# peterhpark/neuroclear

Hardware: AMD Instinct MI355X
Metric: voxels/sec (higher is better)
Workload: dtype f32

## Files before the change

### neuroclear_amd/csrc/norm_act.hip

```cpp
#include <cstdlib>

#include "common.hpp"
#include "s3_common.hpp"

namespace nc {

static constexpr int kMaxSplits = 64;

static int pick_splits(int NC, long S) {
  long want = cdiv(2048, NC);
  long cap = cdiv(S, 8192);
  long s = want < cap ? want : cap;
  if (s < 1) s = 1;
  if (s > kMaxSplits) s = kMaxSplits;
  return (int)s;
}

__device__ __forceinline__ void block_reduce2(double& a, double& b, double* out2) {
  __shared__ double red[2][4];
  for (int o = 32; o > 0; o >>= 1) {
    a += __shfl_down(a, o);
    b += __shfl_down(b, o);
  }
  const int lane = threadIdx.x & 63, wv = threadIdx.x >> 6;
// ... 2 lines not shown
    red[1][wv] = b;
  }
  __syncthreads();
  if (threadIdx.x == 0) {
    out2[0] = (red[0][0] + red[0][1]) + (red[0][2] + red[0][3]);
    out2[1] = (red[1][0] + red[1][1]) + (red[1][2] + red[1][3]);
  }
}

__device__ __forceinline__ void chunk_range(long S, int splits, int sp, long& b, long& e) {
  long chunk = (S + splits - 1) / splits;
  chunk = (chunk + 3) & ~3L;
  b = (long)sp * chunk;
  e = b + chunk < S ? b + chunk : S;
  if (b > S) b = S;
}

__global__ __launch_bounds__(256) void k_in_stats(const float* __restrict__ x, long S, int splits,
                                                  double* __restrict__ part) {
  const int inst = blockIdx.y, sp = blockIdx.x;
  long b, e;
  chunk_range(S, splits, sp, b, e);
  const float* p = x + (long)inst * S;
  double s = 0.0, q = 0.0;
  if ((S & 3) == 0 && ((uintptr_t)x & 15) == 0) {
    const float4* p4 = reinterpret_cast<const float4*>(p);
    for (long i = b / 4 + threadIdx.x; i < e / 4; i += 256) {
      const float4 v = p4[i];
      const double a0 = v.x, a1 = v.y, a2 = v.z, a3 = v.w;
      s += (a0 + a1) + (a2 + a3);
      q = fma(a0, a0, q); q = fma(a1, a1, q); q = fma(a2, a2, q); q = fma(a3, a3, q);
    }
  } else {
    for (long i = b + threadIdx.x; i < e; i += 256) {
      const double a = p[i];
      s += a;
      q = fma(a, a, q);
    }
  }
  block_reduce2(s, q, part + ((long)inst * splits + sp) * 2);
}

__global__ void k_in_finalize(const double* __restrict__ part, int NC, int splits, long S, float eps,
                              float* __restrict__ mean, float* __restrict__ rstd) {
  const int i = blockIdx.x * blockDim.x + threadIdx.x;
  if (i >= NC) return;
  double s = 0.0, q = 0.0;
  for (int k = 0; k < splits; ++k) {
    s += part[((long)i * splits + k) * 2];
    q += part[((long)i * splits + k) * 2 + 1];
  }
  const double m = s / (double)S;
  double var = q / (double)S - m * m;
  if (var < 0.0) var = 0.0;
  mean[i] = (float)m;
  rstd[i] = (float)(1.0 / sqrt(var + (double)eps));
}

__global__ __launch_bounds__(256) void k_in_act_fwd(const float* __restrict__ x, const float* __restrict__ mean,
                                                    const float* __restrict__ rstd, float slope,
                                                    float* __restrict__ y, long S) {
  const int inst = blockIdx.y;
  const float m = mean[inst], r = rstd[inst];
  const float* p = x + (long)inst * S;
  float* o = y + (long)inst * S;
  if ((S & 3) == 0 && (((uintptr_t)x | (uintptr_t)y) & 15) == 0) {
    const float4* p4 = reinterpret_cast<const float4*>(p);
    float4* o4 = reinterpret_cast<float4*>(o);
    for (long i = (long)blockIdx.x * 256 + threadIdx.x; i < S / 4; i += (long)gridDim.x * 256) {
      float4 v = p4[i];
      v.x = (v.x - m) * r; v.y = (v.y - m) * r; v.z = (v.z - m) * r; v.w = (v.w - m) * r;
      v.x = v.x > 0.f ? v.x : v.x * slope; v.y = v.y > 0.f ? v.y : v.y * slope;
      v.z = v.z > 0.f ? v.z : v.z * slope; v.w = v.w > 0.f ? v.w : v.w * slope;
      o4[i] = v;
    }
  } else {
    for (long i = (long)blockIdx.x * 256 + threadIdx.x; i < S; i += (long)gridDim.x * 256) {
      const float v = (p[i] - m) * r;
      o[i] = v > 0.f ? v : v * slope;
    }
  }
}

__global__ __launch_bounds__(256) void k_in_bwd_sums(const float* __restrict__ dy, const float* __restrict__ x,
                                                     const float* __restrict__ mean, const float* __restrict__ rstd,
                                                     float slope, long S, int splits, double* __restrict__ part) {
  const int inst = blockIdx.y, sp = blockIdx.x;
  long b, e;
  chunk_range(S, splits, sp, b, e);
  const float m = mean[inst], r = rstd[inst];
  const float* px = x + (long)inst * S;
  const float* pg = dy + (long)inst * S;
  double s1 = 0.0, s2 = 0.0;
  for (long i = b + threadIdx.x; i < e; i += 256) {
    const float xh = (px[i] - m) * r;
    const float g = xh > 0.f ? pg[i] : pg[i] * slope;
    s1 += (double)g;
    s2 = fma((double)g, (double)xh, s2);
  }
  block_reduce2(s1, s2, part + ((long)inst * splits + sp) * 2);
}

__device__ __forceinline__ float in_bwd_value(float xv, float gy, float m, float r, float m1, float m2, float slope) {
  const float xh = (xv - m) * r;
  const float g = xh > 0.f ? gy : gy * slope;
  float p = xh * m2;
  asm("" : "+v"(p));
  return r * ((g - m1) - p);
}

__global__ __launch_bounds__(256) void k_in_bwd_apply(const float* __restrict__ dy, const float* __restrict__ x,
                                                      const float* __restrict__ mean, const float* __restrict__ rstd,
                                                      float slope, long S, int splits,
                                                      const double* __restrict__ part, float* __restrict__ dx,
                                                      double* __restrict__ rowpart) {
  const int inst = blockIdx.y;
  double s1 = 0.0, s2 = 0.0;
  for (int k = 0; k < splits; ++k) {
    s1 += part[((long)inst * splits + k) * 2];
    s2 += part[((long)inst * splits + k) * 2 + 1];
  }
  const float m1 = (float)(s1 / (double)S), m2 = (float)(s2 / (double)S);
  const float m = mean[inst], r = rstd[inst];
  const float* px = x + (long)inst * S;
  const float* pg = dy + (long)inst * S;
  float* o = dx + (long)inst * S;
  double rs = 0.0;
  for (long i = (long)blockIdx.x * 256 + threadIdx.x; i < S; i += (long)gridDim.x * 256) {
    const float v = in_bwd_value(px[i], pg[i], m, r, m1, m2, slope);
    o[i] = v;
    rs += (double)v;
  }
  if (rowpart) {
    double zero = 0.0, out2[2];
    block_reduce2(rs, zero, out2);
    if (threadIdx.x == 0) rowpart[(long)inst * gridDim.x + blockIdx.x] = out2[0];
  }
}

__global__ __launch_bounds__(256) void k_in_dbias_final(const double* __restrict__ rowpart, int N, int C, int nb,
                                                        float* __restrict__ dbias) {
  const int c = blockIdx.x;
  double s = 0.0, zero = 0.0;
  const int total = N * nb;
  for (int i = threadIdx.x; i < total; i += 256) {
    const int n = i / nb, b = i - n * nb;
    s += rowpart[((long)n * C + c) * nb + b];
  }
  __shared__ double out2[2];
  block_reduce2(s, zero, out2);
  if (threadIdx.x == 0) dbias[c] = (float)out2[0];
}

static constexpr long kRowsMaxS = 2048;

template <int G>
__device__ __forceinline__ double group_sum(double v) {
#pragma unroll
  for (int o = G / 2; o > 0; o >>= 1) v += __shfl_xor(v, o);
  return v;
}

template <int G, int MODE>
__global__ __launch_bounds__(256) void k_in_fwd_rows(const float* __restrict__ x, long NC, int S, float eps, float slope,
                                                     float* __restrict__ mean, float* __restrict__ rstd,
                                                     float* __restrict__ y) {
  const int sub = threadIdx.x % G;
  const long inst = (long)blockIdx.x * (256 / G) + threadIdx.x / G;
  if (inst >= NC) return;
  const float* p = x + inst * S;
  float m, r;
  if constexpr (MODE != 1) {
    double s = 0.0, q = 0.0;
#pragma unroll 4
    for (int i = sub; i < S; i += G) {
      const double a = p[i];
      s += a;
      q = fma(a, a, q);
    }
    s = group_sum<G>(s);
    q = group_sum<G>(q);
    const double mm = s / (double)S;
    double var = q / (double)S - mm * mm;
    if (var < 0.0) var = 0.0;
    m = (float)mm;
    r = (float)(1.0 / sqrt(var + (double)eps));
    if (sub == 0) {
      mean[inst] = m;
      rstd[inst] = r;
    }
  } else {
    m = mean[inst];
    r = rstd[inst];
  }
  if constexpr (MODE != 0) {
    float* o = y + inst * S;
#pragma unroll 4
    for (int i = sub; i < S; i += G) {
      const float v = (p[i] - m) * r;
      o[i] = v > 0.f ? v : v * slope;
    }
  }
}

template <int G>
__global__ __launch_bounds__(256) void k_in_bwd_rows(const float* __restrict__ dy, const float* __restrict__ x,
                                                     const float* __restrict__ mean, const float* __restrict__ rstd,
                                                     float slope, long NC, int S, float* __restrict__ dx,
                                                     double* __restrict__ rowsum) {
  const int sub = threadIdx.x % G;
  const long inst = (long)blockIdx.x * (256 / G) + threadIdx.x / G;
// ... 135 lines not shown
  if (rowpart) {
    const int lane = threadIdx.x & 63, wv = threadIdx.x >> 6;
#pragma unroll
    for (int j = 0; j < 8; ++j) {
      double a = rs[j];
      for (int of = 32; of > 0; of >>= 1) a += __shfl_down(a, of);
      if (lane == 0) red[j][wv] = a;
    }
    __syncthreads();
    if (threadIdx.x < 8)
      rowpart[(ncb * 8 + threadIdx.x) * gridDim.x + blockIdx.x] =
          (red[threadIdx.x][0] + red[threadIdx.x][1]) + (red[threadIdx.x][2] + red[threadIdx.x][3]);
  }
}

__device__ __forceinline__ float r1_product(float w, float s) {
  float g = __builtin_fmaf(w, s, 0.f);
  asm("" : "+v"(g));
  return g;
}

template <bool R1 = false>
__global__ __launch_bounds__(256) void k_in_bwd_apply_s3(const float* __restrict__ dy, const float* __restrict__ x,
                                                         const float* __restrict__ mean, const float* __restrict__ rstd,
                                                         float slope, long S, int splits, const double* __restrict__ part,
                                                         uint4* __restrict__ dxs, int cblocks, double* __restrict__ rowpart,
                                                         const unsigned* __restrict__ guard = nullptr, const float* __restrict__ w1 = nullptr) {
  __shared__ float sm[2][8];
  __shared__ double red[8][4];
  if (guard_skip(guard, 1)) return;
  const long ncb = blockIdx.y;
  if (threadIdx.x < 8) {
    const long inst = ncb * 8 + threadIdx.x;
    double s1 = 0.0, s2 = 0.0;
    for (int k = 0; k < splits; ++k) {
      s1 += part[(inst * splits + k) * 2];
      s2 += part[(inst * splits + k) * 2 + 1];
    }
    sm[0][threadIdx.x] = (float)(s1 / (double)S);
    sm[1][threadIdx.x] = (float)(s2 / (double)S);
  }
  __syncthreads();
  float m[8], r[8], m1[8], m2[8];
#pragma unroll
  for (int j = 0; j < 8; ++j) { m[j] = mean[ncb * 8 + j]; r[j] = rstd[ncb * 8 + j]; m1[j] = sm[0][j]; m2[j] = sm[1][j]; }
  const float* px = x + ncb * 8 * S;
  const float* pg = R1 ? dy : dy + ncb * 8 * S;
  float wj[8];
#pragma unroll
  for (int j = 0; j < 8; ++j) wj[j] = R1 ? w1[ncb * 8 + j] : 0.f;
  double rs[8];
#pragma unroll
  for (int j = 0; j < 8; ++j) rs[j] = 0.0;
  for (long v = (long)blockIdx.x * 256 + threadIdx.x; v < S; v += (long)gridDim.x * 256) {
    unsigned short e[8][3];
    const float sv = R1 ? pg[v] : 0.f;
#pragma unroll
    for (int j = 0; j < 8; ++j) {
      const float t = in_bwd_value(px[j * S + v], R1 ? r1_product(wj[j], sv) : pg[j * S + v], m[j], r[j], m1[j], m2[j], slope);
      rs[j] += (double)t;
      s3_split(t, e[j]);
    }
#pragma unroll
    for (int t = 0; t < 3; ++t) dxs[(ncb * 3 + t) * S + v] = s3_unit(e, t);
  }
  if (rowpart) {
    const int lane = threadIdx.x & 63, wv = threadIdx.x >> 6;
#pragma unroll
    for (int j = 0; j < 8; ++j) {
      double a = rs[j];
      for (int of = 32; of > 0; of >>= 1) a += __shfl_down(a, of);
      if (lane == 0) red[j][wv] = a;
    }
    __syncthreads();
    if (threadIdx.x < 8)
      rowpart[(ncb * 8 + threadIdx.x) * gridDim.x + blockIdx.x] =
          (red[threadIdx.x][0] + red[threadIdx.x][1]) + (red[threadIdx.x][2] + red[threadIdx.x][3]);
  }
}

template <bool R1 = false>
__global__ __launch_bounds__(256) void k_in_bwd_sums_h2(const float* __restrict__ dy, const float* __restrict__ x, const float* __restrict__ mean,
                                                        const float* __restrict__ rstd, float slope, long S, int splits,
                                                        double* __restrict__ part, unsigned* __restrict__ gmax, unsigned* __restrict__ xmax,
                                                        const float* __restrict__ w1 = nullptr) {
  const int inst = blockIdx.y, sp = blockIdx.x;
  long b, e;
  chunk_range(S, splits, sp, b, e);
  const float m = mean[inst], r = rstd[inst];
  const float* px = x + (long)inst * S;
  const float* pg = R1 ? dy : dy + (long)inst * S;
  const float w = R1 ? w1[inst] : 0.f;
  double s1 = 0.0, s2 = 0.0;
  unsigned gm = 0, xm = 0;
  for (long i = b + threadIdx.x; i < e; i += 256) {
    const float xh = (px[i] - m) * r;
    const float gy = R1 ? r1_product(w, pg[i]) : pg[i];
    const float g = xh > 0.f ? gy : gy * slope;
    s1 += (double)g;
    s2 = fma((double)g, (double)xh, s2);
    const unsigned gb = __float_as_uint(g) & 0x7fffffffu, xb = __float_as_uint(xh) & 0x7fffffffu;
    if (gb < 0x7f800000u && gb > gm) gm = gb;
    if (xb < 0x7f800000u && xb > xm) xm = xb;
  }
#pragma unroll
  for (int o = 32; o > 0; o >>= 1) {
    const unsigned q1 = (unsigned)__shfl_xor((int)gm, o), q2 = (unsigned)__shfl_xor((int)xm, o);
    gm = q1 > gm ? q1 : gm; xm = q2 > xm ? q2 : xm;
  }
  if ((threadIdx.x & 63) == 0) {
    if (gm) atomicMax(gmax + inst, gm);
    if (xm) atomicMax(xmax + inst, xm);
  }
  block_reduce2(s1, s2, part + ((long)inst * splits + sp) * 2);
}

__global__ __launch_bounds__(256) void k_in_bwd_bound(const float* __restrict__ rstd, const unsigned* __restrict__ gmax,
                                                      const unsigned* __restrict__ xmax, int NC, unsigned* __restrict__ cell,
                                                      unsigned* __restrict__ cell2, unsigned* __restrict__ guard) {
  if (guard && threadIdx.x < 8) guard[threadIdx.x] = 0u;
  unsigned m = 0;
  for (int i = threadIdx.x; i < NC; i += 256) {
    const float bnd = rstd[i] * __uint_as_float(gmax[i]) * (2.f + __uint_as_float(xmax[i]));
    const unsigned b = __float_as_uint(bnd) & 0x7fffffffu;
    if (b < 0x7f800000u && b > m) m = b;
  }
#pragma unroll
  for (int o = 32; o > 0; o >>= 1) {
    const unsigned q = (unsigned)__shfl_xor((int)m, o);
    m = q > m ? q : m;
  }
  if ((threadIdx.x & 63) == 0 && m) {
    atomicMax(cell, m);
    atomicMax(cell2, m);
  }
}

__global__ void k_zero_u32(unsigned* p, int n) {
  for (int i = blockIdx.x * blockDim.x + threadIdx.x; i < n; i += gridDim.x * blockDim.x) p[i] = 0u;
}

template <bool R1 = false>
__global__ __launch_bounds__(256) void k_in_bwd_apply_h2(const float* __restrict__ dy, const float* __restrict__ x,
                                                         const float* __restrict__ mean, const float* __restrict__ rstd,
                                                         float slope, long S, int splits, const double* __restrict__ part,
                                                         uint4* __restrict__ dxs, int cblocks, double* __restrict__ rowpart,
                                                         const unsigned* __restrict__ cell, unsigned* __restrict__ guard,
                                                         const float* __restrict__ w1 = nullptr) {
  __shared__ float sm[2][8];
  __shared__ double red[8][4];
  const long ncb = blockIdx.y;
  if (threadIdx.x < 8) {
    const long inst = ncb * 8 + threadIdx.x;
    double s1 = 0.0, s2 = 0.0;
    for (int k = 0; k < splits; ++k) {
      s1 += part[(inst * splits + k) * 2];
      s2 += part[(inst * splits + k) * 2 + 1];
    }
    sm[0][threadIdx.x] = (float)(s1 / (double)S);
    sm[1][threadIdx.x] = (float)(s2 / (double)S);
  }
  __syncthreads();
  const unsigned cbits = *cell;
  const float sc = h2_scale(cbits);
  unsigned n_zero = 0, n_low = 0;
  float m[8], r[8], m1[8], m2[8];
#pragma unroll
  for (int j = 0; j < 8; ++j) { m[j] = mean[ncb * 8 + j]; r[j] = rstd[ncb * 8 + j]; m1[j] = sm[0][j]; m2[j] = sm[1][j]; }
  const float* px = x + ncb * 8 * S;
  const float* pg = R1 ? dy : dy + ncb * 8 * S;
  float wj[8];
#pragma unroll
  for (int j = 0; j < 8; ++j) wj[j] = R1 ? w1[ncb * 8 + j] : 0.f;
  double rs[8];
#pragma unroll
  for (int j = 0; j < 8; ++j) rs[j] = 0.0;
  for (long v = (long)blockIdx.x * 256 + threadIdx.x; v < S; v += (long)gridDim.x * 256) {
    unsigned short e[8][3];
    unsigned mx = 0;
    const float sv = R1 ? pg[v] : 0.f;
#pragma unroll
    for (int j = 0; j < 8; ++j) {
      float t = in_bwd_value(px[j * S + v], R1 ? r1_product(wj[j], sv) : pg[j * S + v], m[j], r[j], m1[j], m2[j], slope);
      rs[j] += (double)t;
      asm("" : "+v"(t));
      const unsigned b = __float_as_uint(t) & 0x7fffffffu;
      if (b < 0x7f800000u && b > mx) mx = b;
      h2_split(t * sc, e[j]);
    }
#pragma unroll
    for (int t = 0; t < 2; ++t) dxs[(ncb * 2 + t) * S + v] = s3_unit(e, t);
    if (guard) {
      const unsigned thr = cbits > kGuardDrop ? cbits - kGuardDrop : 0u;
      const bool any_hi = __builtin_amdgcn_ballot_w64(mx >= thr && mx != 0) != 0;
      const bool any_nz = __builtin_amdgcn_ballot_w64(mx != 0) != 0;
      if (!any_nz) ++n_zero;
      else if (!any_hi) ++n_low;
    }
  }
  if (guard && (threadIdx.x & 63) == 0) {
    if (n_low) atomicAdd(guard + kGuardLow, n_low);
    if (n_zero) atomicAdd(guard + kGuardAll, n_zero);
  }
  if (rowpart) {
    const int lane = threadIdx.x & 63, wv = threadIdx.x >> 6;
#pragma unroll
    for (int j = 0; j < 8; ++j) {
      double a = rs[j];
      for (int of = 32; of > 0; of >>= 1) a += __shfl_down(a, of);
      if (lane == 0) red[j][wv] = a;
    }
    __syncthreads();
    if (threadIdx.x < 8)
      rowpart[(ncb * 8 + threadIdx.x) * gridDim.x + blockIdx.x] =
          (red[threadIdx.x][0] + red[threadIdx.x][1]) + (red[threadIdx.x][2] + red[threadIdx.x][3]);
  }
}


__global__ void k_lrelu_fwd(const float* __restrict__ x, float slope, float* __restrict__ y, long n) {
  for (long i = (long)blockIdx.x * blockDim.x + threadIdx.x; i < n; i += (long)gridDim.x * blockDim.x) {
    const float v = x[i];
    y[i] = v > 0.f ? v : v * slope;
  }
}
__global__ void k_lrelu_bwd(const float* __restrict__ dy, const float* __restrict__ x, float slope,
                            float* __restrict__ dx, long n) {
  for (long i = (long)blockIdx.x * blockDim.x + threadIdx.x; i < n; i += (long)gridDim.x * blockDim.x)
    dx[i] = x[i] > 0.f ? dy[i] : dy[i] * slope;
}
__global__ void __launch_bounds__(256) k_in_act_tail(const float* __restrict__ x, const float* __restrict__ mean, const float* __restrict__ rstd,
                                                     const float* __restrict__ w1, const float* __restrict__ b1, const float* __restrict__ w2,
                                                     const float* __restrict__ b2, float* __restrict__ y, long S, int C) {
  __shared__ float sm[3][256];
  for (int c = threadIdx.x; c < C; c += 256) { sm[0][c] = mean[c]; sm[1][c] = rstd[c]; sm[2][c] = w1[c]; }
  __syncthreads();
  const long v = (long)blockIdx.x * 256 + threadIdx.x;
  if (v >= S) return;
  float acc = 0.f;
  for (int c = 0; c < C; ++c) {
    float t = (x[(long)c * S + v] - sm[0][c]) * sm[1][c];
    t = t > 0.f ? t : 0.f;
    acc = fmaf(sm[2][c], t, acc);
  }
  const float t1 = acc + b1[0];
  const float t2 = fmaf(w2[0], t1, b2[0]);
// ... 186 lines not shown
                      void* stream) {
  if (!x || !mean || !rstd) { set_error("instnorm_stats: null pointer"); return NC_ERR_ARG; }
  if (NC >= 1 && S >= 1 && rows_path(S)) {
    launch_fwd_rows<0>(x, NC, S, eps, 0.f, mean, rstd, nullptr, (hipStream_t)stream);
    return check_launch("instnorm_stats");
  }
  if (NC > 65535) {
    for (int c0 = 0; c0 < NC; c0 += 65535) {
      const int n = NC - c0 < 65535 ? NC - c0 : 65535;
      if (int e = nc_instnorm_stats(x + (long)c0 * S, n, S, eps, mean + c0, rstd + c0, ws, ws_bytes, stream)) return e;
    }
    return NC_OK;
  }
  if (NC < 1 || S < 1) { set_error("instnorm_stats: bad shape NC=%d S=%ld", NC, S); return NC_ERR_SHAPE; }
  if (!ws || ws_bytes < nc_instnorm_ws_bytes(NC, S)) { set_error("instnorm_stats: workspace too small"); return NC_ERR_WS; }
  hipStream_t s = (hipStream_t)stream;
  const int splits = pick_splits(NC, S);
  hipLaunchKernelGGL(k_in_stats, dim3(splits, NC), dim3(256), 0, s, x, S, splits, (double*)ws);
  hipLaunchKernelGGL(k_in_finalize, dim3((unsigned)cdiv(NC, 128)), dim3(128), 0, s, (const double*)ws, NC, splits, S, eps,
                     mean, rstd);
  return check_launch("instnorm_stats");
}

int nc_instnorm_act_fwd(const float* x, const float* mean, const float* rstd, float slope, float* y, int NC, long S,
                        void* stream) {
  if (!x || !mean || !rstd || !y) { set_error("instnorm_act_fwd: null pointer"); return NC_ERR_ARG; }
  if (NC >= 1 && S >= 1 && rows_path(S)) {
    launch_fwd_rows<1>(x, NC, S, 0.f, slope, const_cast<float*>(mean), const_cast<float*>(rstd), y, (hipStream_t)stream);
    return check_launch("instnorm_act_fwd");
  }
  if (NC > 65535) {
    for (int c0 = 0; c0 < NC; c0 += 65535) {
      const int n = NC - c0 < 65535 ? NC - c0 : 65535;
      if (int e = nc_instnorm_act_fwd(x + (long)c0 * S, mean + c0, rstd + c0, slope, y + (long)c0 * S, n, S, stream)) return e;
    }
    return NC_OK;
  }
  if (NC < 1 || S < 1) { set_error("instnorm_act_fwd: bad shape"); return NC_ERR_SHAPE; }
  long bx = cdiv(S, 1024 * 4);
  if (bx > 1024) bx = 1024;
  hipLaunchKernelGGL(k_in_act_fwd, dim3((unsigned)bx, NC), dim3(256), 0, (hipStream_t)stream, x, mean, rstd, slope, y, S);
  return check_launch("instnorm_act_fwd");
}

int nc_instnorm_fwd(const float* x, float eps, float slope, float* mean, float* rstd, float* y, int NC, long S, void* ws,
                    size_t ws_bytes, void* stream) {
  if (!x || !mean || !rstd || !y) { set_error("instnorm_fwd: null pointer"); return NC_ERR_ARG; }
  if (NC < 1 || S < 1) { set_error("instnorm_fwd: bad shape NC=%d S=%ld", NC, S); return NC_ERR_SHAPE; }
  if (rows_path(S)) {
    launch_fwd_rows<2>(x, NC, S, eps, slope, mean, rstd, y, (hipStream_t)stream);
    return check_launch("instnorm_fwd");
  }
  if (int e = nc_instnorm_stats(x, NC, S, eps, mean, rstd, ws, ws_bytes, stream)) return e;
  return nc_instnorm_act_fwd(x, mean, rstd, slope, y, NC, S, stream);
}

int nc_instnorm_act_bwd(const float* dy, const float* x, const float* mean, const float* rstd, float slope, float* dx,
                        int NC, long S, void* ws, size_t ws_bytes, void* stream) {
  if (!dy || !x || !mean || !rstd || !dx) { set_error("instnorm_act_bwd: null pointer"); return NC_ERR_ARG; }
  if (NC >= 1 && S >= 1 && rows_path(S)) {
    launch_bwd_rows(dy, x, mean, rstd, slope, NC, S, dx, nullptr, (hipStream_t)stream);
    return check_launch("instnorm_act_bwd");
  }
  if (NC > 65535) {
    for (int c0 = 0; c0 < NC; c0 += 65535) {
      const int n = NC - c0 < 65535 ? NC - c0 : 65535;
      if (int e = nc_instnorm_act_bwd(dy + (long)c0 * S, x + (long)c0 * S, mean + c0, rstd + c0, slope, dx + (long)c0 * S, n, S, ws,
                                      ws_bytes, stream)) return e;
    }
    return NC_OK;
  }
  if (NC < 1 || S < 1) { set_error("instnorm_act_bwd: bad shape"); return NC_ERR_SHAPE; }
  if (!ws || ws_bytes < nc_instnorm_ws_bytes(NC, S)) { set_error("instnorm_act_bwd: workspace too small"); return NC_ERR_WS; }
  hipStream_t s = (hipStream_t)stream;
  const int splits = pick_splits(NC, S);
  hipLaunchKernelGGL(k_in_bwd_sums, dim3(splits, NC), dim3(256), 0, s, dy, x, mean, rstd, slope, S, splits, (double*)ws);
  long bx = cdiv(S, 1024);
  if (bx > 1024) bx = 1024;
  hipLaunchKernelGGL(k_in_bwd_apply, dim3((unsigned)bx, NC), dim3(256), 0, s, dy, x, mean, rstd, slope, S, splits,
                     (const double*)ws, dx, (double*)nullptr);
  return check_launch("instnorm_act_bwd");
}

size_t nc_instnorm_bwd_dbias_ws_bytes(int NC, long S) {
  long bx = cdiv(S, 1024);
  if (bx > 1024) bx = 1024;
  return nc_instnorm_ws_bytes(NC, S) + (size_t)NC * bx * sizeof(double);
}

int nc_instnorm_act_bwd_dbias(const float* dy, const float* x, const float* mean, const float* rstd, float slope, float* dx,
                              float* dbias, int N, int C, long S, void* ws, size_t ws_bytes, void* stream) {
  if (!dy || !x || !mean || !rstd || !dx || !dbias) { set_error("instnorm_act_bwd_dbias: null pointer"); return NC_ERR_ARG; }
  const long NCl = (long)N * C;
  if (N < 1 || C < 1 || S < 1 || NCl > 0x7fffffffL) { set_error("instnorm_act_bwd_dbias: bad shape"); return NC_ERR_SHAPE; }
  hipStream_t s = (hipStream_t)stream;
  if (rows_path(S)) {
    if (!ws || ws_bytes < (size_t)NCl * sizeof(double)) { set_error("instnorm_act_bwd_dbias: workspace too small"); return NC_ERR_WS; }
    launch_bwd_rows(dy, x, mean, rstd, slope, NCl, S, dx, (double*)ws, s);
    hipLaunchKernelGGL(k_in_dbias_final, dim3(C), dim3(256), 0, s, (const double*)ws, N, C, 1, dbias);
    return check_launch("instnorm_act_bwd_dbias");
  }
  if (NCl > 65535) { set_error("instnorm_act_bwd_dbias: more than 65535 long instances"); return NC_ERR_SHAPE; }
  const int NC = (int)NCl;
  if (!ws || ws_bytes < nc_instnorm_bwd_dbias_ws_bytes(NC, S)) { set_error("instnorm_act_bwd_dbias: workspace too small"); return NC_ERR_WS; }
  const int splits = pick_splits(NC, S);
  double* rowpart = (double*)((char*)ws + nc_instnorm_ws_bytes(NC, S));
  hipLaunchKernelGGL(k_in_bwd_sums, dim3(splits, NC), dim3(256), 0, s, dy, x, mean, rstd, slope, S, splits, (double*)ws);
  long bx = cdiv(S, 1024);
  if (bx > 1024) bx = 1024;
  hipLaunchKernelGGL(k_in_bwd_apply, dim3((unsigned)bx, NC), dim3(256), 0, s, dy, x, mean, rstd, slope, S, splits,
                     (const double*)ws, dx, rowpart);
  hipLaunchKernelGGL(k_in_dbias_final, dim3(C), dim3(256), 0, s, (const double*)rowpart, N, C, (int)bx, dbias);
  return check_launch("instnorm_act_bwd_dbias");
}

int nc_instnorm_act_fwd_c8(const float* x, const float* mean, const float* rstd, float slope, float* y, void* yh, int N, int C,
                           long S, int dtype, void* stream) {
  if (!x || !mean || !rstd || !yh) { set_error("instnorm_act_fwd_c8: null pointer"); return NC_ERR_ARG; }
  if (N < 1 || C < 8 || C % 8 || S < 1 || (long)N * C / 8 > 65535) { set_error("instnorm_act_fwd_c8: bad shape"); return NC_ERR_SHAPE; }
  if (dtype != NC_DT_F16 && dtype != NC_DT_BF16) { set_error("instnorm_act_fwd_c8: dtype must be NC_DT_F16 or NC_DT_BF16"); return NC_ERR_ARG; }
  long bx = cdiv(S, 256);
  if (bx > 2048) bx = 2048;
  dim3 grid((unsigned)bx, (unsigned)(N * C / 8));
  if (dtype == NC_DT_F16)
    hipLaunchKernelGGL(k_in_act_fwd_c8<NC_DT_F16>, grid, dim3(256), 0, (hipStream_t)stream, x, mean, rstd, slope, y, (uint4*)yh, S);
  else
    hipLaunchKernelGGL(k_in_act_fwd_c8<NC_DT_BF16>, grid, dim3(256), 0, (hipStream_t)stream, x, mean, rstd, slope, y, (uint4*)yh, S);
  return check_launch("instnorm_act_fwd_c8");
}

int nc_instnorm_act_bwd_c8(const float* dy, const float* x, const float* mean, const float* rstd, float slope, float* dx,
                           void* dxh, float* dbias, int N, int C, long S, int dtype, void* ws, size_t ws_bytes, void* stream) {
  if (!dy || !x || !mean || !rstd || !dx || !dxh) { set_error("instnorm_act_bwd_c8: null pointer"); return NC_ERR_ARG; }
  const long NCl = (long)N * C;
  if (N < 1 || C < 8 || C % 8 || S < 1 || NCl > 65535) { set_error("instnorm_act_bwd_c8: bad shape"); return NC_ERR_SHAPE; }
  if (dtype != NC_DT_F16 && dtype != NC_DT_BF16) { set_error("instnorm_act_bwd_c8: dtype must be NC_DT_F16 or NC_DT_BF16"); return NC_ERR_ARG; }
  const int NC = (int)NCl;
  if (!ws || ws_bytes < nc_instnorm_bwd_dbias_ws_bytes(NC, S)) { set_error("instnorm_act_bwd_c8: workspace too small"); return NC_ERR_WS; }
  hipStream_t s = (hipStream_t)stream;
  const int splits = pick_splits(NC, S);
  hipLaunchKernelGGL(k_in_bwd_sums, dim3(splits, NC), dim3(256), 0, s, dy, x, mean, rstd, slope, S, splits, (double*)ws);
  long bx = cdiv(S, 1024);
  if (bx > 1024) bx = 1024;
  double* rowpart = dbias ? (double*)((char*)ws + nc_instnorm_ws_bytes(NC, S)) : nullptr;
  dim3 grid((unsigned)bx, (unsigned)(NC / 8));
  if (dtype == NC_DT_F16)
    hipLaunchKernelGGL(k_in_bwd_apply_c8<NC_DT_F16>, grid, dim3(256), 0, s, dy, x, mean, rstd, slope, S, splits,
                       (const double*)ws, dx, (uint4*)dxh, rowpart);
  else
    hipLaunchKernelGGL(k_in_bwd_apply_c8<NC_DT_BF16>, grid, dim3(256), 0, s, dy, x, mean, rstd, slope, S, splits,
                       (const double*)ws, dx, (uint4*)dxh, rowpart);
  if (dbias) hipLaunchKernelGGL(k_in_dbias_final, dim3(C), dim3(256), 0, s, (const double*)rowpart, N, C, (int)bx, dbias);
  return check_launch("instnorm_act_bwd_c8");
}

}
namespace nc {
bool instnorm_bwd_s3_supported(int N, int C, long S) { return N >= 1 && C >= 8 && C % 8 == 0 && S >= 1 && !rows_path(S) && (long)N * C <= 65535; }
int instnorm_act_bwd_dbias_s3(const float* dy, const float* x, const float* mean, const float* rstd, float slope, void* dxs,
                              float* dbias, int N, int C, long S, void* ws, size_t ws_bytes, void* stream) {
  if (!dy || !x || !mean || !rstd || !dxs || !dbias) { set_error("instnorm_act_bwd_dbias_s3: null pointer"); return NC_ERR_ARG; }
  if (!instnorm_bwd_s3_supported(N, C, S)) { set_error("instnorm_act_bwd_dbias_s3: bad shape"); return NC_ERR_SHAPE; }
  const int NC = N * C;
  if (!ws || ws_bytes < nc_instnorm_bwd_dbias_ws_bytes(NC, S)) { set_error("instnorm_act_bwd_dbias_s3: workspace too small"); return NC_ERR_WS; }
  hipStream_t s = (hipStream_t)stream;
  const int splits = pick_splits(NC, S);
  hipLaunchKernelGGL(k_in_bwd_sums, dim3(splits, NC), dim3(256), 0, s, dy, x, mean, rstd, slope, S, splits, (double*)ws);
  long bx = cdiv(S, 1024);
  if (bx > 1024) bx = 1024;
  double* rowpart = (double*)((char*)ws + nc_instnorm_ws_bytes(NC, S));
  hipLaunchKernelGGL(k_in_bwd_apply_s3<false>, dim3((unsigned)bx, (unsigned)(NC / 8)), dim3(256), 0, s, dy, x, mean, rstd, slope, S, splits,
                     (const double*)ws, (uint4*)dxs, C / 8, rowpart, (const unsigned*)nullptr, (const float*)nullptr);
  hipLaunchKernelGGL(k_in_dbias_final, dim3(C), dim3(256), 0, s, (const double*)rowpart, N, C, (int)bx, dbias);
  return check_launch("instnorm_act_bwd_dbias_s3");
}
static int in_bwd_dbias_h2(const float* dy, const float* w1, const float* x, const float* mean, const float* rstd, float slope, void* dxs,
                           float* dbias, int N, int C, long S, void* ws, size_t ws_bytes, void* stream, unsigned* guard) {
  if (!dy || !x || !mean || !rstd || !dxs || !dbias) { set_error("instnorm_act_bwd_dbias_h2: null pointer"); return NC_ERR_ARG; }
  if (!instnorm_bwd_s3_supported(N, C, S)) { set_error("instnorm_act_bwd_dbias_h2: bad shape"); return NC_ERR_SHAPE; }
  const int NC = N * C;
  if (w1 && N != 1) { set_error("instnorm_act_bwd_dbias_h2: the rank-one form takes one sample"); return NC_ERR_ARG; }
  if (!ws || ws_bytes < nc_instnorm_bwd_dbias_ws_bytes(NC, S)) { set_error("instnorm_act_bwd_dbias_h2: workspace too small"); return NC_ERR_WS; }
  if ((size_t)NC * S * 2 < 512 + (size_t)NC * 8) { set_error("instnorm_act_bwd_dbias_h2: tensor too small"); return NC_ERR_SHAPE; }
  hipStream_t s = (hipStream_t)stream;
  unsigned* cells = (unsigned*)((char*)dxs + h2_cells_offset((size_t)NC * S));
  unsigned* gmax = cells + 64;
  unsigned* xmax = gmax + NC;
  hipLaunchKernelGGL(k_zero_u32, dim3((unsigned)cdiv(64 + 2 * NC, 256)), dim3(256), 0, s, cells, 64 + 2 * NC);
  const int splits = pick_splits(NC, S);
  if (w1)
    hipLaunchKernelGGL(k_in_bwd_sums_h2<true>, dim3(splits, NC), dim3(256), 0, s, dy, x, mean, rstd, slope, S, splits, (double*)ws, gmax, xmax, w1);
  else
    hipLaunchKernelGGL(k_in_bwd_sums_h2<false>, dim3(splits, NC), dim3(256), 0, s, dy, x, mean, rstd, slope, S, splits, (double*)ws, gmax, xmax,
                       (const float*)nullptr);
  hipLaunchKernelGGL(k_in_bwd_bound, dim3(1), dim3(256), 0, s, rstd, gmax, xmax, NC, cells, cells + 1, guard);
  long bx = cdiv(S, 1024);
  if (bx > 1024) bx = 1024;
  double* rowpart = (double*)((char*)ws + nc_instnorm_ws_bytes(NC, S));
  unsigned* g = guard && h2_guard_on() ? guard : nullptr;
  if (w1)
    hipLaunchKernelGGL(k_in_bwd_apply_h2<true>, dim3((unsigned)bx, (unsigned)(NC / 8)), dim3(256), 0, s, dy, x, mean, rstd, slope, S, splits,
                       (const double*)ws, (uint4*)dxs, C / 8, rowpart, (const unsigned*)cells, g, w1);
  else
    hipLaunchKernelGGL(k_in_bwd_apply_h2<false>, dim3((unsigned)bx, (unsigned)(NC / 8)), dim3(256), 0, s, dy, x, mean, rstd, slope, S, splits,
                       (const double*)ws, (uint4*)dxs, C / 8, rowpart, (const unsigned*)cells, g, (const float*)nullptr);
  hipLaunchKernelGGL(k_in_dbias_final, dim3(C), dim3(256), 0, s, (const double*)rowpart, N, C, (int)bx, dbias);
  if (g) {
    const unsigned long long total = (unsigned long long)(NC / 8) * (unsigned long long)cdiv(S, 64);
    const bool flip = h2_guard_can_flip();
    if (int e = h2_guard_decide(g, nullptr, nullptr, g + kGuardFlag, flip, s, total)) return e;
    if (!flip) return check_launch("instnorm_act_bwd_dbias_h2");
    long bx3 = bx < 128 ? bx : 128;
    if (w1)
      hipLaunchKernelGGL(k_in_bwd_apply_s3<true>, dim3((unsigned)bx3, (unsigned)(NC / 8)), dim3(256), 0, s, dy, x, mean, rstd, slope, S, splits,
                         (const double*)ws, (uint4*)dxs, C / 8, (double*)nullptr, (const unsigned*)g, w1);
    else
      hipLaunchKernelGGL(k_in_bwd_apply_s3<false>, dim3((unsigned)bx3, (unsigned)(NC / 8)), dim3(256), 0, s, dy, x, mean, rstd, slope, S, splits,
                         (const double*)ws, (uint4*)dxs, C / 8, (double*)nullptr, (const unsigned*)g, (const float*)nullptr);
  }
  return check_launch("instnorm_act_bwd_dbias_h2");
}
int instnorm_act_bwd_dbias_h2(const float* dy, const float* x, const float* mean, const float* rstd, float slope, void* dxs,
                              float* dbias, int N, int C, long S, void* ws, size_t ws_bytes, void* stream, unsigned* guard) {
  return in_bwd_dbias_h2(dy, nullptr, x, mean, rstd, slope, dxs, dbias, N, C, S, ws, ws_bytes, stream, guard);
}
int instnorm_act_bwd_dbias_h2_rank1(const float* dy1, const float* w1, const float* x, const float* mean, const float* rstd, float slope, void* dxs,
                                    float* dbias, int C, long S, void* ws, size_t ws_bytes, void* stream, unsigned* guard) {
  if (!w1) { set_error("instnorm_act_bwd_dbias_h2_rank1: null pointer"); return NC_ERR_ARG; }
  return in_bwd_dbias_h2(dy1, w1, x, mean, rstd, slope, dxs, dbias, 1, C, S, ws, ws_bytes, stream, guard);
}
int instnorm_relu_tail_sigmoid(const float* x, const float* mean, const float* rstd, const float* w1, const float* b1, const float* w2,
                               const float* b2, float* y, int C, long S, hipStream_t s) {
  if (C > 256) { set_error("instnorm_relu_tail_sigmoid: at most 256 channels"); return NC_ERR_SHAPE; }
  hipLaunchKernelGGL(k_in_act_tail, dim3((unsigned)cdiv(S, 256)), dim3(256), 0, s, x, mean, rstd, w1, b1, w2, b2, y, S, C);
  return check_launch("instnorm_relu_tail_sigmoid");
}
}
extern "C" {

int nc_instnorm_act_bwd_dbias_s3(const float* dy, const float* x, const float* mean, const float* rstd, float slope, void* dxs, float* dbias,
                                 int N, int C, long S, void* ws, size_t ws_bytes, void* stream) {
  return instnorm_act_bwd_dbias_s3(dy, x, mean, rstd, slope, dxs, dbias, N, C, S, ws, ws_bytes, stream);
}

int nc_leaky_relu_fwd(const float* x, float slope, float* y, long n, void* stream) {
  if (!x || !y) { set_error("leaky_relu_fwd: null pointer"); return NC_ERR_ARG; }
  hipLaunchKernelGGL(k_lrelu_fwd, dim3(flat_grid(n)), dim3(256), 0, (hipStream_t)stream, x, slope, y, n);
  return check_launch("leaky_relu_fwd");
}
int nc_leaky_relu_bwd(const float* dy, const float* x, float slope, float* dx, long n, void* stream) {
  if (!dy || !x || !dx) { set_error("leaky_relu_bwd: null pointer"); return NC_ERR_ARG; }
  hipLaunchKernelGGL(k_lrelu_bwd, dim3(flat_grid(n)), dim3(256), 0, (hipStream_t)stream, dy, x, slope, dx, n);
  return check_launch("leaky_relu_bwd");
}
int nc_sigmoid_fwd(const float* x, float* y, long n, void* stream) {
  if (!x || !y) { set_error("sigmoid_fwd: null pointer"); return NC_ERR_ARG; }
  hipLaunchKernelGGL(k_sigmoid_fwd, dim3(flat_grid(n)), dim3(256), 0, (hipStream_t)stream, x, y, n);
  return check_launch("sigmoid_fwd");
}
int nc_sigmoid_bwd(const float* dy, const float* y, float* dx, long n, void* stream) {
  if (!dy || !y || !dx) { set_error("sigmoid_bwd: null pointer"); return NC_ERR_ARG; }
  hipLaunchKernelGGL(k_sigmoid_bwd, dim3(flat_grid(n)), dim3(256), 0, (hipStream_t)stream, dy, y, dx, n);
  return check_launch("sigmoid_bwd");
}

int nc_maxpool2_fwd(const float* x, float* y, int NC, int D, int H, int W, void* stream) {
  if (!x || !y) { set_error("maxpool2_fwd: null pointer"); return NC_ERR_ARG; }
  const int wd = D > 1 ? 2 : 1;
  const int Do = D / wd, Ho = H / 2, Wo = W / 2;
  if (NC < 1 || Do < 1 || Ho < 1 || Wo < 1) { set_error("maxpool2_fwd: bad shape"); return NC_ERR_SHAPE; }
  const long total = (long)NC * Do * Ho * Wo;
  hipLaunchKernelGGL(k_maxpool2_fwd, dim3(flat_grid(total)), dim3(256), 0, (hipStream_t)stream, x, y, NC, D, H, W, Do, Ho, Wo, wd);
  return check_launch("maxpool2_fwd");
}

int nc_maxpool2_bwd(const float* dy, const float* x, float* dx, int NC, int D, int H, int W, void* stream) {
  if (!dy || !x || !dx) { set_error("maxpool2_bwd: null pointer"); return NC_ERR_ARG; }
  const int wd = D > 1 ? 2 : 1;
  const int Do = D / wd, Ho = H / 2, Wo = W / 2;
  if (NC < 1 || Do < 1 || Ho < 1 || Wo < 1) { set_error("maxpool2_bwd: bad shape"); return NC_ERR_SHAPE; }
  hipStream_t s = (hipStream_t)stream;
  if ((D % wd) || (H & 1) || (W & 1)) {
    if (hipMemsetAsync(dx, 0, (size_t)NC * D * H * W * sizeof(float), s) != hipSuccess) {
      set_error("maxpool2_bwd: memset failed");
      return NC_ERR_HIP;
    }
  }
  const long total = (long)NC * Do * Ho * Wo;
// ... 78 lines not shown
```

Measured before the change: 54.99 million.

## Unroll instance-norm backward loops and fold max-bound kernel into apply kernel

Unrolls the sum and apply loops of instance-norm backward so each thread issues several independent loads before computing. The h2 path drops the zero-fill kernel and the single-block bound kernel. It writes per-split gradient and activation maxima to workspace instead of using atomics, and every apply block recomputes the global bound from those maxima. This removes two launches and the atomic traffic. In exchange each apply block does a redundant reduction over NC×splits entries, and the workspace grows.

```diff
diff --git a/neuroclear_amd/csrc/norm_act.hip b/neuroclear_amd/csrc/norm_act.hip
--- a/neuroclear_amd/csrc/norm_act.hip
+++ b/neuroclear_amd/csrc/norm_act.hip
@@ -108,6 +108,14 @@
   }
 }
 
+static constexpr int kInSumsU = 8, kInApplyU = 4;
+
+template <int U>
+__device__ __forceinline__ void load_group(const float* __restrict__ p, long i, long stride, float (&v)[U]) {
+#pragma unroll
+  for (int u = 0; u < U; ++u) v[u] = p[i + u * stride];
+}
+
 __global__ __launch_bounds__(256) void k_in_bwd_sums(const float* __restrict__ dy, const float* __restrict__ x,
                                                      const float* __restrict__ mean, const float* __restrict__ rstd,
                                                      float slope, long S, int splits, double* __restrict__ part) {
@@ -118,12 +126,21 @@
   const float* px = x + (long)inst * S;
   const float* pg = dy + (long)inst * S;
   double s1 = 0.0, s2 = 0.0;
-  for (long i = b + threadIdx.x; i < e; i += 256) {
-    const float xh = (px[i] - m) * r;
-    const float g = xh > 0.f ? pg[i] : pg[i] * slope;
+  auto acc = [&](float xv, float gv) {
+    const float xh = (xv - m) * r;
+    const float g = xh > 0.f ? gv : gv * slope;
     s1 += (double)g;
     s2 = fma((double)g, (double)xh, s2);
-  }
+  };
+  long i = b + threadIdx.x;
+  for (; i + (kInSumsU - 1) * 256 < e; i += kInSumsU * 256) {
+    float xv[kInSumsU], gv[kInSumsU];
+    load_group(px, i, 256, xv);
+    load_group(pg, i, 256, gv);
+#pragma unroll
+    for (int u = 0; u < kInSumsU; ++u) acc(xv[u], gv[u]);
+  }
+  for (; i < e; i += 256) acc(px[i], pg[i]);
   block_reduce2(s1, s2, part + ((long)inst * splits + sp) * 2);
 }
 
@@ -152,7 +169,20 @@
   const float* pg = dy + (long)inst * S;
   float* o = dx + (long)inst * S;
   double rs = 0.0;
-  for (long i = (long)blockIdx.x * 256 + threadIdx.x; i < S; i += (long)gridDim.x * 256) {
+  const long step = (long)gridDim.x * 256;
+  long i = (long)blockIdx.x * 256 + threadIdx.x;
+  for (; i + (kInApplyU - 1) * step < S; i += kInApplyU * step) {
+    float xv[kInApplyU], gv[kInApplyU];
+    load_group(px, i, step, xv);
+    load_group(pg, i, step, gv);
+#pragma unroll
+    for (int u = 0; u < kInApplyU; ++u) {
+      const float v = in_bwd_value(xv[u], gv[u], m, r, m1, m2, slope);
+      o[i + u * step] = v;
+      rs += (double)v;
+    }
+  }
+  for (; i < S; i += step) {
     const float v = in_bwd_value(px[i], pg[i], m, r, m1, m2, slope);
     o[i] = v;
     rs += (double)v;
@@ -454,9 +484,10 @@
 template <bool R1 = false>
 __global__ __launch_bounds__(256) void k_in_bwd_sums_h2(const float* __restrict__ dy, const float* __restrict__ x, const float* __restrict__ mean,
                                                         const float* __restrict__ rstd, float slope, long S, int splits,
-                                                        double* __restrict__ part, unsigned* __restrict__ gmax, unsigned* __restrict__ xmax,
+                                                        double* __restrict__ part, unsigned* __restrict__ maxes, unsigned* __restrict__ guard,
                                                         const float* __restrict__ w1 = nullptr) {
   const int inst = blockIdx.y, sp = blockIdx.x;
+  if (guard && inst == 0 && sp == 0 && threadIdx.x < 8) guard[threadIdx.x] = 0u;
   long b, e;
   chunk_range(S, splits, sp, b, e);
   const float m = mean[inst], r = rstd[inst];
@@ -465,51 +496,72 @@
   const float w = R1 ? w1[inst] : 0.f;
   double s1 = 0.0, s2 = 0.0;
   unsigned gm = 0, xm = 0;
-  for (long i = b + threadIdx.x; i < e; i += 256) {
-    const float xh = (px[i] - m) * r;
-    const float gy = R1 ? r1_product(w, pg[i]) : pg[i];
+  auto acc = [&](float xv, float gv) {
+    const float xh = (xv - m) * r;
+    const float gy = R1 ? r1_product(w, gv) : gv;
     const float g = xh > 0.f ? gy : gy * slope;
     s1 += (double)g;
     s2 = fma((double)g, (double)xh, s2);
     const unsigned gb = __float_as_uint(g) & 0x7fffffffu, xb = __float_as_uint(xh) & 0x7fffffffu;
     if (gb < 0x7f800000u && gb > gm) gm = gb;
     if (xb < 0x7f800000u && xb > xm) xm = xb;
-  }
+  };
+  long i = b + threadIdx.x;
+  for (; i + (kInSumsU - 1) * 256 < e; i += kInSumsU * 256) {
+    float xv[kInSumsU], gv[kInSumsU];
+    load_group(px, i, 256, xv);
+    load_group(pg, i, 256, gv);
+#pragma unroll
+    for (int u = 0; u < kInSumsU; ++u) acc(xv[u], gv[u]);
+  }
+  for (; i < e; i += 256) acc(px[i], pg[i]);
 #pragma unroll
   for (int o = 32; o > 0; o >>= 1) {
     const unsigned q1 = (unsigned)__shfl_xor((int)gm, o), q2 = (unsigned)__shfl_xor((int)xm, o);
     gm = q1 > gm ? q1 : gm; xm = q2 > xm ? q2 : xm;
   }
-  if ((threadIdx.x & 63) == 0) {
-    if (gm) atomicMax(gmax + inst, gm);
-    if (xm) atomicMax(xmax + inst, xm);
-  }
+  __shared__ unsigned mx[2][4];
+  if ((threadIdx.x & 63) == 0) { mx[0][threadIdx.x >> 6] = gm; mx[1][threadIdx.x >> 6] = xm; }
   block_reduce2(s1, s2, part + ((long)inst * splits + sp) * 2);
-}
-
-__global__ __launch_bounds__(256) void k_in_bwd_bound(const float* __restrict__ rstd, const unsigned* __restrict__ gmax,
-                                                      const unsigned* __restrict__ xmax, int NC, unsigned* __restrict__ cell,
-                                                      unsigned* __restrict__ cell2, unsigned* __restrict__ guard) {
-  if (guard && threadIdx.x < 8) guard[threadIdx.x] = 0u;
+  if (threadIdx.x < 2) {
+    const unsigned* q = mx[threadIdx.x];
+    const unsigned a = q[0] > q[1] ? q[0] : q[1], c = q[2] > q[3] ? q[2] : q[3];
+    maxes[((long)inst * splits + sp) * 2 + threadIdx.x] = a > c ? a : c;
+  }
+}
+
+__device__ __forceinline__ unsigned in_bwd_bound(const float* __restrict__ rstd, const unsigned* __restrict__ maxes, int NC, int splits) {
+  __shared__ unsigned wm[4];
   unsigned m = 0;
-  for (int i = threadIdx.x; i < NC; i += 256) {
-    const float bnd = rstd[i] * __uint_as_float(gmax[i]) * (2.f + __uint_as_float(xmax[i]));
-    const unsigned b = __float_as_uint(bnd) & 0x7fffffffu;
-    if (b < 0x7f800000u && b > m) m = b;
+  const int sub = threadIdx.x & 3;
+  for (int i0 = 0; i0 < NC; i0 += 64) {
+    const int i = i0 + (threadIdx.x >> 2);
+    unsigned gm = 0, xm = 0;
+    if (i < NC)
+      for (int k = sub; k < splits; k += 4) {
+        const unsigned g = maxes[((long)i * splits + k) * 2], xh = maxes[((long)i * splits + k) * 2 + 1];
+        gm = g > gm ? g : gm; xm = xh > xm ? xh : xm;
+      }
+#pragma unroll
+    for (int o = 1; o < 4; o <<= 1) {
+      const unsigned q1 = (unsigned)__shfl_xor((int)gm, o), q2 = (unsigned)__shfl_xor((int)xm, o);
+      gm = q1 > gm ? q1 : gm; xm = q2 > xm ? q2 : xm;
+    }
+    if (i < NC) {
+      const float bnd = rstd[i] * __uint_as_float(gm) * (2.f + __uint_as_float(xm));
+      const unsigned b = __float_as_uint(bnd) & 0x7fffffffu;
+      if (b < 0x7f800000u && b > m) m = b;
+    }
   }
 #pragma unroll
   for (int o = 32; o > 0; o >>= 1) {
     const unsigned q = (unsigned)__shfl_xor((int)m, o);
     m = q > m ? q : m;
   }
-  if ((threadIdx.x & 63) == 0 && m) {
-    atomicMax(cell, m);
-    atomicMax(cell2, m);
-  }
-}
-
-__global__ void k_zero_u32(unsigned* p, int n) {
-  for (int i = blockIdx.x * blockDim.x + threadIdx.x; i < n; i += gridDim.x * blockDim.x) p[i] = 0u;
+  if ((threadIdx.x & 63) == 0) wm[threadIdx.x >> 6] = m;
+  __syncthreads();
+  const unsigned a = wm[0] > wm[1] ? wm[0] : wm[1], c = wm[2] > wm[3] ? wm[2] : wm[3];
+  return a > c ? a : c;
 }
 
 template <bool R1 = false>
@@ -517,8 +569,8 @@
                                                          const float* __restrict__ mean, const float* __restrict__ rstd,
                                                          float slope, long S, int splits, const double* __restrict__ part,
                                                          uint4* __restrict__ dxs, int cblocks, double* __restrict__ rowpart,
-                                                         const unsigned* __restrict__ cell, unsigned* __restrict__ guard,
-                                                         const float* __restrict__ w1 = nullptr) {
+                                                         const unsigned* __restrict__ maxes, unsigned* __restrict__ cells,
+                                                         unsigned* __restrict__ guard, const float* __restrict__ w1 = nullptr) {
   __shared__ float sm[2][8];
   __shared__ double red[8][4];
   const long ncb = blockIdx.y;
@@ -533,7 +585,8 @@
     sm[1][threadIdx.x] = (float)(s2 / (double)S);
   }
   __syncthreads();
-  const unsigned cbits = *cell;
+  const unsigned cbits = in_bwd_bound(rstd, maxes, (int)gridDim.y * 8, splits);
+  if (blockIdx.x == 0 && blockIdx.y == 0 && threadIdx.x < 2) cells[threadIdx.x] = cbits;
   const float sc = h2_scale(cbits);
   unsigned n_zero = 0, n_low = 0;
   float m[8], r[8], m1[8], m2[8];
@@ -886,10 +939,13 @@
   return check_launch("instnorm_act_bwd");
 }
 
-size_t nc_instnorm_bwd_dbias_ws_bytes(int NC, long S) {
+static size_t in_bwd_maxes_offset(int NC, long S) {
   long bx = cdiv(S, 1024);
   if (bx > 1024) bx = 1024;
   return nc_instnorm_ws_bytes(NC, S) + (size_t)NC * bx * sizeof(double);
+}
+size_t nc_instnorm_bwd_dbias_ws_bytes(int NC, long S) {
+  return in_bwd_maxes_offset(NC, S) + (size_t)NC * kMaxSplits * 2 * sizeof(unsigned);
 }
 
 int nc_instnorm_act_bwd_dbias(const float* dy, const float* x, const float* mean, const float* rstd, float slope, float* dx,
@@ -985,29 +1041,26 @@
   const int NC = N * C;
   if (w1 && N != 1) { set_error("instnorm_act_bwd_dbias_h2: the rank-one form takes one sample"); return NC_ERR_ARG; }
   if (!ws || ws_bytes < nc_instnorm_bwd_dbias_ws_bytes(NC, S)) { set_error("instnorm_act_bwd_dbias_h2: workspace too small"); return NC_ERR_WS; }
-  if ((size_t)NC * S * 2 < 512 + (size_t)NC * 8) { set_error("instnorm_act_bwd_dbias_h2: tensor too small"); return NC_ERR_SHAPE; }
+  if ((size_t)NC * S * 2 < 512) { set_error("instnorm_act_bwd_dbias_h2: tensor too small"); return NC_ERR_SHAPE; }
   hipStream_t s = (hipStream_t)stream;
   unsigned* cells = (unsigned*)((char*)dxs + h2_cells_offset((size_t)NC * S));
-  unsigned* gmax = cells + 64;
-  unsigned* xmax = gmax + NC;
-  hipLaunchKernelGGL(k_zero_u32, dim3((unsigned)cdiv(64 + 2 * NC, 256)), dim3(256), 0, s, cells, 64 + 2 * NC);
+  unsigned* maxes = (unsigned*)((char*)ws + in_bwd_maxes_offset(NC, S));
   const int splits = pick_splits(NC, S);
   if (w1)
-    hipLaunchKernelGGL(k_in_bwd_sums_h2<true>, dim3(splits, NC), dim3(256), 0, s, dy, x, mean, rstd, slope, S, splits, (double*)ws, gmax, xmax, w1);
+    hipLaunchKernelGGL(k_in_bwd_sums_h2<true>, dim3(splits, NC), dim3(256), 0, s, dy, x, mean, rstd, slope, S, splits, (double*)ws, maxes, guard, w1);
   else
-    hipLaunchKernelGGL(k_in_bwd_sums_h2<false>, dim3(splits, NC), dim3(256), 0, s, dy, x, mean, rstd, slope, S, splits, (double*)ws, gmax, xmax,
+    hipLaunchKernelGGL(k_in_bwd_sums_h2<false>, dim3(splits, NC), dim3(256), 0, s, dy, x, mean, rstd, slope, S, splits, (double*)ws, maxes, guard,
                        (const float*)nullptr);
-  hipLaunchKernelGGL(k_in_bwd_bound, dim3(1), dim3(256), 0, s, rstd, gmax, xmax, NC, cells, cells + 1, guard);
   long bx = cdiv(S, 1024);
   if (bx > 1024) bx = 1024;
   double* rowpart = (double*)((char*)ws + nc_instnorm_ws_bytes(NC, S));
   unsigned* g = guard && h2_guard_on() ? guard : nullptr;
   if (w1)
     hipLaunchKernelGGL(k_in_bwd_apply_h2<true>, dim3((unsigned)bx, (unsigned)(NC / 8)), dim3(256), 0, s, dy, x, mean, rstd, slope, S, splits,
-                       (const double*)ws, (uint4*)dxs, C / 8, rowpart, (const unsigned*)cells, g, w1);
+                       (const double*)ws, (uint4*)dxs, C / 8, rowpart, (const unsigned*)maxes, cells, g, w1);
   else
     hipLaunchKernelGGL(k_in_bwd_apply_h2<false>, dim3((unsigned)bx, (unsigned)(NC / 8)), dim3(256), 0, s, dy, x, mean, rstd, slope, S, splits,
-                       (const double*)ws, (uint4*)dxs, C / 8, rowpart, (const unsigned*)cells, g, (const float*)nullptr);
+                       (const double*)ws, (uint4*)dxs, C / 8, rowpart, (const unsigned*)maxes, cells, g, (const float*)nullptr);
   hipLaunchKernelGGL(k_in_dbias_final, dim3(C), dim3(256), 0, s, (const double*)rowpart, N, C, (int)bx, dbias);
   if (g) {
     const unsigned long long total = (unsigned long long)(NC / 8) * (unsigned long long)cdiv(S, 64);
```

New measurement: 55.40 million (median of 6 runs). About the same (+0.8%).
